# vshiv18/khoice

Measured on AMD Instinct MI355X. Metric: distinct k-mers/sec (k=31, canonical), higher is better.
Workload: dtype u64

## Files before the change

### khoice_amd/csrc/kh_engine.cpp

```cpp
#include <hip/hip_runtime.h>

#include <algorithm>
#include <atomic>
#include <thread>
#include <chrono>
#include <cmath>
#include <memory>
#include <cstdarg>
#include <cstdio>
#include <cstdlib>
#include <cstring>
#include <map>
#include <mutex>
#include <string>
#include <vector>

#include "../../include/khoice_hip.h"
#include "kh_engine.h"
#include "kh_launch.h"
#include "kh_skm_rec.h"

static thread_local std::string g_last_error;

int kh_fail(int code, const char* fmt, ...) {
// ... 344 lines not shown
extern "C" int kh_set_counts(kh_ctx* c, const kh_set* in, uint32_t value, kh_set** out) {
    if (!c || !in || !out) return kh_fail(KH_E_ARG, "kh_set_counts: NULL argument");
    if (value == 0) return kh_fail(KH_E_ARG, "set_counts 0 would empty the database");
    buf_ref(in->kb);
    *out = make_set(in->k, in->n, in->kb, in->koff, nullptr, 0, value, std::max<u32>(value, KH_KMC_DEFAULT_CS));
    return KH_OK;
}

#ifdef KH_STAMPS
void kh_debug_set_stamps(u64* p);
void kh_debug_set_stamps_skm(u64* p);
static void report_stamps(kh_ctx* c, const char* what, DevBuf* sb, u64 nparts) {
    std::vector<u64> h(nparts * 16);
    (void)hipMemcpyAsync(h.data(), sb->p, nparts * 128, hipMemcpyDeviceToHost, c->st);
    (void)hipStreamSynchronize(c->st);
    double sum[16] = {0};
    u64 cnt = 0, tmin = ~0ull, tmax = 0;
    for (u64 q = 0; q < nparts; ++q) {
        const u64* t = &h[q * 16];
        if (!t[0] || !t[8]) continue;
        ++cnt;
        for (int i = 1; i <= 8; ++i) if (t[i] && t[i - 1]) sum[i] += (double)(t[i] - t[i - 1]);
        tmin = std::min(tmin, t[0]);
        tmax = std::max(tmax, t[8]);
    }
    {
        double s9 = 0, s10 = 0, s11 = 0; u64 c9 = 0;
        for (u64 q = 0; q < nparts; ++q) {
            const u64* t = &h[q * 16];
            if (!t[4] || !t[9] || !t[10] || !t[11] || !t[5]) continue;
            ++c9; s9 += (double)(t[9] - t[4]); s10 += (double)(t[10] - t[9]); s11 += (double)(t[11] - t[10]);
        }
        if (c9) fprintf(stderr, "[stamps] %s inside 4-5: first-probe %.0f rounds %.0f stores %.0f (then barrier)\n", what, s9 / c9, s10 / c9, s11 / c9);
    }
    fprintf(stderr, "[stamps] %s parts=%llu span=%.0f cyc | load %.0f count %.0f scan %.0f scatter %.0f insert %.0f walk1 %.0f lookback %.0f walk2 %.0f\n",
            what, (unsigned long long)cnt, (double)(tmax - tmin), sum[1] / cnt, sum[2] / cnt, sum[3] / cnt, sum[4] / cnt,
            sum[5] / cnt, sum[6] / cnt, sum[7] / cnt, sum[8] / cnt);
    {
        std::string line;
        for (int i = 1; i < 16; ++i) {
            double s2 = 0; u64 c2 = 0;
            for (u64 q = 0; q < nparts; ++q) {
                const u64* t = &h[q * 16];
                if (!t[0] || !t[i]) continue;
                ++c2; s2 += (double)((long long)(t[i] - t[0]));
            }
            if (c2) { char b[64]; snprintf(b, sizeof b, " t%d=%.0f(n=%llu)", i, s2 / c2, (unsigned long long)c2); line += b; }
        }
        fprintf(stderr, "[stamps] %s offsets from t0:%s\n", what, line.c_str());
    }
}
#ifdef KH_STAMPS_WG
void kh_debug_set_stamps_skm2(u64* p);
static void dump_wg_ends(kh_ctx* c, DevBuf* sb, u32 grid) {
    const char* path = getenv("KHOICE_WG_DUMP");
    if (!path) return;
    static int call = 0;
    std::vector<u64> h((size_t)grid * 16);
    (void)hipMemcpyAsync(h.data(), sb->p, (size_t)grid * 128, hipMemcpyDeviceToHost, c->st);
    (void)hipStreamSynchronize(c->st);
    FILE* f = fopen(path, "a");
    if (!f) return;
    for (u32 b = 0; b < grid; ++b) {
        const u64* t = &h[(size_t)b * 16];
        fprintf(f, "%d %u %llu %llu %llu %llu %llu %llu\n", call, b, (unsigned long long)t[1], (unsigned long long)t[2],
                (unsigned long long)t[0], (unsigned long long)t[8], (unsigned long long)t[3], (unsigned long long)t[11]);
    }
    fclose(f);
    ++call;
}
#endif
#endif

struct TextStage {
    Tmp d_seq;
    std::vector<const u8*> dev;
    int copy_in(kh_ctx* c, int n, const uint8_t* const* seqs, const uint64_t* lens, int on_device, const int* perm = nullptr) {
        auto in_place = [&](const uint8_t* p) { return on_device && (reinterpret_cast<uintptr_t>(p) & 15) == 0; };
        std::vector<u64> pack_off(n);
        u64 seq_bytes = 0;
        bool need_pack = false;
        for (int i = 0; i < n; ++i) {
            const int t = perm ? perm[i] : i;
            pack_off[i] = seq_bytes;
            seq_bytes += (lens[t] + 15) & ~15ull;
            if (!in_place(seqs[t])) need_pack = true;
        }
        TMP_ALLOC(d_seq, c, need_pack ? seq_bytes + 256 : 256);
        dev.resize(n);
        for (int i = 0; i < n; ++i) {
            const int t = perm ? perm[i] : i;
            if (in_place(seqs[t])) { dev[i] = seqs[t]; continue; }
            dev[i] = d_seq.as<u8>() + pack_off[i];
            if (!lens[t]) continue;
            HIPCHK(hipMemcpyAsync(d_seq.as<u8>() + pack_off[i], seqs[t], lens[t],
                                  on_device ? hipMemcpyDeviceToDevice : hipMemcpyHostToDevice, c->st));
            c->stat.text_packed += lens[t];
        }
        return KH_OK;
    }
};

struct GridBuild {
    kh_ctx* c = nullptr;
    u32 fan = 1;
    u32 cap = 0;
    double s_scale = 1.0;
    u32 wave = 0, nwaves = 1;
    u32 nb = 0, S = 0, nb_total = 0;
    u64 total_pos = 0, bases = 0, key_cap = 0;
// ... 1176 lines not shown
    const u64 lim = (u64)wd.max_coarse * wd.max_fine;
    if (!force_slots && nslots64 > lim) {
        const double per_slot = (double)positions * per_kmer / (double)lim;
        const double s2 = ((double)max_cap2 - 112.0) / per_slot;
        if (s2 >= 1.4 && (!g.two || (double)positions / (double)lim <= 0.75 * (double)wd.table)) {
            nslots64 = lim;
            slack2 = std::min(slack2, s2);
        }
    }
    const u32 max_coarse = nslots64 > lim ? kh_skm_width(true).max_coarse : wd.max_coarse;
    if (nslots64 > (u64)max_coarse * wd.max_fine) {
        if (!table || force_slots) return false;
        nslots64 = (u64)max_coarse * wd.max_fine;
        fuller = true;
    }
    g.nslots = (u32)nslots64;
    g.S = std::max<u32>(1, (g.nslots + max_coarse - 1) / max_coarse);
    g.nb1 = (g.nslots + g.S - 1) / g.S;
    const double recs = (double)positions * per_kmer;
    if (const char* e = getenv("KHOICE_SKM_SLACK")) slack1 = slack2 = std::max(0.01, atof(e));
    const u64 cap1_64 = ((u64)(recs / g.nb1 * slack1) + 2048 + 63) & ~63ull;
    u64 cap2_64 = ((u64)(recs / g.nslots * slack2) + 96 + 15) & ~15ull;
    if (cap2_64 > max_cap2 && !force_slots && !fuller) {
        if ((double)fan + recs / (double)g.nslots <= (double)max_cap2 - 112.0) cap2_64 = max_cap2 & ~15u;
    }
    if (cap2_64 > max_cap2 || cap1_64 > 0x7fffffffull) return false;
    g.cap1 = (u32)cap1_64;
    g.cap2 = (u32)cap2_64;
    g.ugrid = std::min<u32>(g.nslots, wd.union_per_cu * (u32)std::max(1, cus));
    *out = g;
    return true;
}
template <class F> static int timed_launch(kh_ctx* c, int cls, F launch) {
    c->prof_begin(cls);
    launch();
    c->prof_end();
    HIPCHK(hipGetLastError());
    return KH_OK;
}
struct SkmRun {
    kh_ctx* c;
    TagLayout L;
    SkmGeometry g;
    KhSkmJob job;
    struct Layout { size_t ctl, inst, dup, cur1, cur2, claim, ginfo, tags, segs, tiles, bytes; } off{};
    TextStage texts;
    Tmp d_ws, d_reg1, d_reg2, d_spill;
    Pinned pin;
    u8* h_down = nullptr;
    u32 ntiles = 0;
    u64 bases = 0;
    bool staged = false;
    static constexpr u32 spill_cap = 1u << 20, big_cap = 16384u;
#ifdef KH_STAMPS
    Tmp d_stamps;
#endif
    explicit SkmRun(kh_ctx* ctx) : c(ctx), pin{ctx} {}

    void layout(size_t hist_words, int nseq) {
        off.ctl = 8 * hist_words;
        off.inst = off.ctl + 4 * (size_t)KH_SKM_CTL_WORDS;
        off.dup = off.inst + 8 * (size_t)nseq;
        off.cur1 = off.dup + 8 * 64;
        off.cur2 = off.cur1 + 4 * (size_t)KH_SKM_CUR1_STRIDE * g.nb1;
        off.claim = (off.cur2 + 4 * (size_t)g.nslots + 127) & ~(size_t)127;
        off.ginfo = off.claim + 128;
        off.tags = off.ginfo + 256;
        off.segs = off.tags + (((size_t)nseq + 15) & ~(size_t)15);
        off.tiles = off.segs + sizeof(KhSeg) * nseq;
        off.bytes = off.tiles + sizeof(KhTile) * (size_t)std::max<u32>(1, ntiles);
    }
    template <class T> T* dev(size_t o) const { return reinterpret_cast<T*>(d_ws.as<u8>() + o); }
    int read_back(size_t from) {
        HIPCHK(hipMemcpyAsync(h_down + from, d_ws.as<u8>() + from, off.cur1 - from, hipMemcpyDeviceToHost, c->st));
        HIPCHK(hipStreamSynchronize(c->st));
        return KH_OK;
    }
    const u64* h_hist() const { return reinterpret_cast<const u64*>(h_down); }
    const u32* h_ctl() const { return reinterpret_cast<const u32*>(h_down + off.ctl); }
    const u64* h_inst() const { return reinterpret_cast<const u64*>(h_down + off.inst); }
    const u64* h_dup() const { return reinterpret_cast<const u64*>(h_down + off.dup); }
    bool failed() const { return (h_ctl()[KH_SKM_CTL_ERR] & (KH_ERR_CAPACITY | KH_ERR_ORDER)) != 0; }
    template <class F> int settle(size_t from, F listed, bool* declines) {
        *declines = true;
        KHCHK(read_back(from));
        const u32* hc = h_ctl();
        if (hc[KH_SKM_CTL_LISTED] && !failed()) {
            if (hc[KH_SKM_CTL_SPILLED] > spill_cap || hc[KH_SKM_CTL_LISTED] > big_cap) { c->stat.retries++; return KH_OK; }
            KHCHK(listed(hc[KH_SKM_CTL_LISTED]));
            KHCHK(read_back(from));
        }
        if (failed()) { c->stat.retries++; return KH_OK; }
        *declines = false;
        return KH_OK;
    }
    template <class F> void per_text(F f) const {
        for (int i = 0; i < L.nseq; ++i) f(L.perm[i], h_inst()[i], h_inst()[i] - h_dup()[i]);
    }
};
static int skm_prepare(kh_ctx* c, int nseq, const uint8_t* const* seqs, const uint64_t* lens, int on_device,
                       const int* group_of, int ngroups, int k, bool by_group, u32 force_slots, u32 fan_hint, SkmRun* s,
                       u32 table = 0 ) {
    TagLayout* L = &s->L;
    if (!skm_form_k(k)) return KH_OK;
    if ((!by_group && nseq > KH_TAG_MAX_OPS) || ngroups > KH_TAG_MAX_OPS) return KH_OK;
    KHCHK(tag_layout(L, nseq, group_of, ngroups, by_group));
    if (L->nbins > (u32)KH_TAG_MAX_BINS) return KH_OK;
    const u64 positions = kmer_positions(nseq, lens, k, &s->bases);
    if (!skm_plan(k, positions, std::max(L->fan, fan_hint), force_slots, c->cus, &s->g, table)) return KH_OK;
    const SkmGeometry& g = s->g;
    const KhSkmWidth& wd = *g.wd;
    const size_t rec_bytes = wd.rec_bytes;
    const size_t reg1_bytes = rec_bytes * (size_t)g.nb1 * g.cap1, reg2_bytes = rec_bytes * (size_t)g.nslots * g.cap2;
    HIPCHK(hipSetDevice(c->dev));
    {
        size_t free_b = 0, total_b = 0;
        if (hipMemGetInfo(&free_b, &total_b) == hipSuccess &&
            reg1_bytes + reg2_bytes + s->bases + (64u << 20) > free_b + c->pool.cached_bytes)
            return KH_OK;
    }
    hipStream_t st = c->st;

    u32 tile_pos = KH_TILE;
    {
        const u64 want_tiles = 8ull * (u64)std::max(1, c->cus);
        while (tile_pos > (u32)KH_SUBTILE && (positions + tile_pos - 1) / tile_pos < want_tiles) tile_pos >>= 1;
    }
    std::vector<KhSeg> segs(nseq);
    std::vector<KhTile> tiles;
    for (int i = 0; i < nseq; ++i) {
        KhSeg& sg = segs[i];
        memset(&sg, 0, sizeof sg);
        const u64 len = lens[L->perm[i]];
        sg.len = len;
        sg.npos = len >= (u64)k ? len - k + 1 : 0;
        sg.ntiles = (u32)((sg.npos + tile_pos - 1) / tile_pos);
        sg.tile_base = (u32)tiles.size();
        for (u32 t = 0; t < sg.ntiles; ++t) tiles.push_back(KhTile{(u32)i, t});
    }
    const u32 ntiles = s->ntiles = (u32)tiles.size();
    const u32 reps = g.ugrid;
    s->layout((size_t)reps * L->nbins, nseq);
    const SkmRun::Layout& off = s->off;
    const u32 spill_cap = SkmRun::spill_cap;
    TMP_ALLOC(s->d_ws, c, off.bytes);
    TMP_ALLOC(s->d_reg1, c, reg1_bytes);
    TMP_ALLOC(s->d_reg2, c, reg2_bytes);
    TMP_ALLOC(s->d_spill, c, (size_t)spill_cap * (rec_bytes + 4) + (size_t)SkmRun::big_cap * 4);
    const size_t up_bytes = off.bytes - off.ginfo;
    PIN_ALLOC(s->pin, up_bytes + off.cur1 + 64);
    u8* h_up = static_cast<u8*>(s->pin.p);
    s->h_down = h_up + ((up_bytes + 63) & ~(size_t)63);
    c->prof_begin(KC_COPY_IN);
    KHCHK(s->texts.copy_in(c, nseq, seqs, lens, on_device, L->perm.data()));
    for (int i = 0; i < nseq; ++i) segs[i].seq = s->texts.dev[i];
    memcpy(h_up + (off.segs - off.ginfo), segs.data(), sizeof(KhSeg) * nseq);
    if (ntiles) memcpy(h_up + (off.tiles - off.ginfo), tiles.data(), sizeof(KhTile) * (size_t)ntiles);
    L->words(reinterpret_cast<u32*>(h_up), h_up + (off.tags - off.ginfo), group_of);
    HIPCHK(hipMemsetAsync(s->d_ws.b->p, 0, off.ginfo, st));
    HIPCHK(hipMemcpyAsync(s->dev<u8>(off.ginfo), h_up, up_bytes, hipMemcpyHostToDevice, st));
    c->prof_end();

    KhSkmJob& job = s->job;
    job.seg_tag = by_group ? s->dev<const u8>(off.tags) : nullptr;
    job.segs = s->dev<const KhSeg>(off.segs);
    job.tiles = s->dev<const KhTile>(off.tiles);
    job.reg1 = s->d_reg1.as<uint4>();
    job.reg2 = s->d_reg2.as<uint4>();
    job.cur1 = s->dev<u32>(off.cur1);
    job.cur2 = s->dev<u32>(off.cur2);
    job.inst = s->dev<unsigned long long>(off.inst);
    job.dup = s->dev<unsigned long long>(off.dup);
    job.ginfo = s->dev<const u32>(off.ginfo);
    job.hist = s->dev<unsigned long long>(0);
    job.ctl = s->dev<u32>(off.ctl);
    job.claim = s->dev<u32>(off.claim);
    job.tile_pos = tile_pos;
    job.k = k; job.m = g.m; job.w = g.w; job.nmax = g.nmax;
    job.nslots = g.nslots; job.S = g.S; job.nb1 = g.nb1; job.cap1 = g.cap1; job.cap2 = g.cap2;
    job.nbins = L->nbins; job.abase = L->abase; job.reps = reps; job.nops = by_group ? (u32)ngroups : (u32)nseq;
    job.spill_rec = s->d_spill.as<uint4>();
    job.spill_slot = reinterpret_cast<u32*>(s->d_spill.as<u8>() + (size_t)spill_cap * rec_bytes);
    job.big_list = reinterpret_cast<u32*>(s->d_spill.as<u8>() + (size_t)spill_cap * (rec_bytes + 4));
    job.spill_cap = spill_cap;
    job.big_cap = SkmRun::big_cap;
#ifdef KH_STAMPS
    const u64 nst = std::max<u64>(ntiles, g.nslots);
    TMP_ALLOC(s->d_stamps, c, 128 * nst);
    HIPCHK(hipMemsetAsync(s->d_stamps.b->p, 0, 128 * nst, st));
    kh_debug_set_stamps_skm(s->d_stamps.as<u64>());
#endif
    c->prof_begin(KC_SKM_SCATTER);
    wd.scatter(job, ntiles, st);
    c->prof_end();
#ifdef KH_STAMPS
    report_stamps(c, "skm_scatter (second sub-tile: codes / hashes / minima / slots+count / - / append / barrier / -)", s->d_stamps.b, ntiles);
    HIPCHK(hipMemsetAsync(s->d_stamps.b->p, 0, 128 * nst, st));
    kh_debug_set_stamps_skm(nullptr);
#endif
    c->prof_begin(KC_SKM_REGROUP);
    wd.regroup(job, st);
    c->prof_end();
#ifdef KH_STAMPS
    kh_debug_set_stamps_skm(s->d_stamps.as<u64>());
#ifdef KH_STAMPS_WG
    kh_debug_set_stamps_skm2(s->d_stamps.as<u64>());
#endif
#endif
    s->staged = true;
    return KH_OK;
}
static int exp1_skm(kh_ctx* c, const Exp1In& in, uint64_t* within_hist, uint64_t* across_hist, uint64_t* distinct_per_seq,
                    bool* done, bool by_group = false) {
    *done = false;
    SkmRun s(c);
    KHCHK(skm_prepare(c, in.nseq, in.seqs, in.lens, in.on_device, in.group_of, in.ngroups, in.k, by_group, 0, 0, &s));
    if (!s.staged) return KH_OK;
    const TagLayout& L = s.L;
    const SkmGeometry& g = s.g;
    const KhSkmJob& job = s.job;
    hipStream_t st = c->st;
    KHCHK(timed_launch(c, KC_SKM_UNION, [&] { g.wd->unite(job, in.cs, g.ugrid, st); }));
#if defined(KH_STAMPS) && defined(KH_STAMPS_WG)
    dump_wg_ends(c, s.d_stamps.b, g.ugrid);
    kh_debug_set_stamps_skm(nullptr);
    kh_debug_set_stamps_skm2(nullptr);
#elif defined(KH_STAMPS)
    report_stamps(c, "skm_union (scan barrier / owner / expand / insert / barrier / read-out / barrier / flush)", s.d_stamps.b, g.nslots);
    kh_debug_set_stamps_skm(nullptr);
#endif
    if (getenv("KHOICE_SKM_DEBUG")) {
        std::vector<u32> h1(g.nb1), h2(g.nslots);
        HIPCHK(hipMemcpy2DAsync(h1.data(), 4, job.cur1, 4 * (size_t)KH_SKM_CUR1_STRIDE, 4, g.nb1, hipMemcpyDeviceToHost, st));
        HIPCHK(hipMemcpyAsync(h2.data(), job.cur2, 4 * (size_t)g.nslots, hipMemcpyDeviceToHost, st));
        u32 hc[KH_SKM_CTL_WORDS];
        HIPCHK(hipMemcpyAsync(hc, job.ctl, sizeof hc, hipMemcpyDeviceToHost, st));
        HIPCHK(hipStreamSynchronize(st));
        u64 t1 = 0, t2 = 0;
        u32 m1 = 0, m2 = 0;
        for (u32 v : h1) { t1 += v; m1 = std::max(m1, v); }
        for (u32 v : h2) { t2 += v; m2 = std::max(m2, v); }
        fprintf(stderr, "[skm] k=%d m=%d w=%u nmax=%u positions=%llu records=%llu (%.2f k-mers each) nb1=%u S=%u nslots=%u | "
                        "coarse: mean %.0f max %u cap %u | slot: mean %.1f max %u cap %u | tiles %u x %u | expanded: %u k-mers | errors %u spilled %u overfull slots %u multi-subset slots %u tail-wide waves %u\n",
                in.k, g.m, g.w, g.nmax, (unsigned long long)g.positions, (unsigned long long)t1, (double)g.positions / std::max<u64>(1, t1),
                g.nb1, g.S, g.nslots, (double)t1 / g.nb1, m1, g.cap1, (double)t2 / g.nslots, m2, g.cap2, s.ntiles, job.tile_pos,
                hc[KH_SKM_CTL_EXPANDED], hc[KH_SKM_CTL_ERR], hc[KH_SKM_CTL_SPILLED], hc[KH_SKM_CTL_LISTED], g.two ? 0u : hc[KH_SKM_CTL_MULTI], g.two ? 0u : hc[KH_SKM_CTL_TAILWIDE]);
    }
    bool declines = false;
// ... 1920 lines not shown
```

### khoice_amd/csrc/kh_launch.h

```cpp
#pragma once
#include <hip/hip_runtime.h>
#include "kh_common.h"

struct KhSeg {
    const u8* seq;
    u64 len;
    u64 npos;
    u64 thist_base;
    u32 nbuckets;
    u32 bucket_base;
    u32 tile_base;
    u32 ntiles;
    u32 nb_virtual;
    u32 b_first;
};
struct KhTile { u32 seg; u32 tile_in_seg; };

struct KhBucketWork {
    u64 lo;
    u64 out_base;
    u32 n;
    u32 nb;
    u32 b;
    u32 gb;
// ... 89 lines not shown
    uint4* reg2;
    u32* cur1;
    u32* cur2;
    unsigned long long* inst;
    unsigned long long* dup;
    const u32* ginfo;
    unsigned long long* hist;
    u32* ctl;
    u32* claim;
    u32 tile_pos;
    int k, m;
    u32 w;
    u32 nmax;
    u32 nslots, S, nb1, cap1, cap2;
    u32 nbins, abase, reps, nops;
    uint4* spill_rec;
    u32* spill_slot;
    u32* big_list;
    u32 spill_cap, big_cap;
};
struct KhSkmCrossJob {
    unsigned long long* bins;
    u32 pmlo, pmhi;
    u32 ngenomes;
    u32 nbins, reps;
    u32 nlisted;
};
struct KhSkmPivotJob {
    KhSkmCrossJob cj;
    u32 pinfo[KH_TAG_MAX_OPS];
};
constexpr int KH_SKM2_MAX_K = 63;
constexpr u32 KH_SKM2_MAX_COARSE = 512;
constexpr u32 KH_SKM2_MAX_FINE = 1024;
struct KhSkmWidth {
    u32 rec_bytes;
    u32 max_coarse, max_fine;
    u32 max_cap2;
    u32 table;
    u32 union_per_cu, cross_per_cu;
    u32 pivot_per_cu;
    u32 cross_round;
    bool (*supports_w)(u32 w);
    void (*scatter)(const KhSkmJob& job, u32 ntiles, hipStream_t st);
    void (*regroup)(const KhSkmJob& job, hipStream_t st);
    void (*unite)(const KhSkmJob& job, u32 cs, u32 grid, hipStream_t st);
    void (*big)(const KhSkmJob& job, u32 cs, u32 nbig, hipStream_t st);
    void (*cross)(const KhSkmJob& job, const KhSkmCrossJob& cj, u32 grid, hipStream_t st);
    void (*pivot)(const KhSkmJob& job, const KhSkmPivotJob& pj, u32 grid, hipStream_t st);
};
const KhSkmWidth& kh_skm_width1();
const KhSkmWidth& kh_skm_width2();
inline const KhSkmWidth& kh_skm_width(bool two) { return two ? kh_skm_width2() : kh_skm_width1(); }
struct KhSkmPackJob {
    const uint4* reg2;
    const u32* cur2;
    uint4* out_rec;
    u32* out_mask;
    u32* part_cursor;
    u32* slot_count;
    u32* slot_off;
    u32* ctl;
    unsigned long long* dup;
    u64 part_cap;
    u32 cap2, nslots, spp;
    u32 nsub;
};
struct KhSkmCompactJob {
    const uint4* tmp_rec;
    const u32* tmp_mask;
    uint4* out_rec;
    u32* out_mask;
    const u32* cursors;
    u32* slot_off;
    u32* part_n;
    u64 part_cap;
    u32 nslots, spp, nsub, nparts;
};
void kh_launch_skm_pack_compact(const KhSkmCompactJob& job, hipStream_t st);
struct KhSkmPiece {
    const uint4* rec;
    const u32* mask;
    const u32* count;
    const u32* off;
    u32 dup_row;
    u32 join_next;
};
struct KhSkmPhasedJob {
    const KhSkmPiece* pieces;
    unsigned long long* hist;
    u32* ctl;
    unsigned long long* dup;
    u32 npieces, nslots, hist_len, cs;
    u32 share_q8;
    int k;
};
constexpr u32 KH_SKM_PHASED_MAX_DUP_PIECES = 32;
size_t kh_skm_phased_lds_bytes();
void kh_launch_skm_pack(const KhSkmPackJob& job, hipStream_t st);
void kh_launch_skm_phased(const KhSkmPhasedJob& job, u32 grid, hipStream_t st);

#ifndef KH_TUNE_BMP_RANGE_BITS
#define KH_TUNE_BMP_RANGE_BITS 20
#endif
constexpr int KH_BMP_RANGE_BITS = KH_TUNE_BMP_RANGE_BITS;
constexpr int KH_BMP_MAX_K = 12;
// ... 137 lines not shown
```

### khoice_amd/csrc/kh_skm.hip

```cpp
#include <hip/hip_runtime.h>

#include "kh_device.h"
#include "kh_launch.h"

#ifdef KH_STAMPS
__device__ u64* g_skm_stamps = nullptr;
void kh_debug_set_stamps_skm(u64* p) { (void)hipMemcpyToSymbol(HIP_SYMBOL(g_skm_stamps), &p, sizeof p); }
#define SKM_STAMP(idx)                                                                     \
    do {                                                                                   \
        __builtin_amdgcn_sched_barrier(0);                                                 \
        if (threadIdx.x == 0 && g_skm_stamps)                                              \
            g_skm_stamps[((u64)blockIdx.y * gridDim.x + blockIdx.x) * 16 + (idx)] = __builtin_amdgcn_s_memtime(); \
        __builtin_amdgcn_sched_barrier(0);                                                 \
    } while (0)
#else
#define SKM_STAMP(idx) do {} while (0)
#endif

#ifdef KH_MARKS
#define SKM_MARK(name) asm volatile("; ===== MARK " name ::: "memory")
#else
#define SKM_MARK(name) do {} while (0)
#endif
#ifndef KH_TUNE_SKM_SCATTER_PREFETCH
#define KH_TUNE_SKM_SCATTER_PREFETCH 0
#endif
#ifndef KH_TUNE_SKM_SCATTER_WAVES
#define KH_TUNE_SKM_SCATTER_WAVES 3
#endif

#include "kh_skm_device.h"

static size_t kh_skm_scatter_lds_bytes(u32 nb1) {
    const u32 nbk = (nb1 + 3) & ~3u;
    return flush_lds_bytes<SKM_CAP>(nbk) + (size_t)SKM_CW * 4 + (((size_t)SKM_CW * 2 + 15) & ~(size_t)15) + 64 * 4 + 4 * 32 * 4 +
           (size_t)SKM_NT * 8 + 64;
}

template <int WW>
__global__ __launch_bounds__(SKM_NT, KH_TUNE_SKM_SCATTER_WAVES) void k_skm_scatter(const KhSkmJob jb) {
    extern __shared__ __attribute__((aligned(16))) u8 lds_raw[];
    const u32 nbk = (jb.nb1 + 3) & ~3u;
    const FlushLds L = flush_lds<SKM_CAP>(lds_raw, nbk);
    u8* p = lds_raw + flush_lds_bytes<SKM_CAP>(nbk);
    u32* code = reinterpret_cast<u32*>(p);                    p += (size_t)SKM_CW * 4;
    u16* bad16 = reinterpret_cast<u16*>(p);                   p += ((size_t)SKM_CW * 2 + 15) & ~(size_t)15;
    u32* tailh = reinterpret_cast<u32*>(p);                   p += 64 * 4;
    u32* xch = reinterpret_cast<u32*>(p);                     p += 4 * 32 * 4;
    uint2* lrun = reinterpret_cast<uint2*>(p);                p += (size_t)SKM_NT * 8;
    u32* misc = reinterpret_cast<u32*>(p);

    const u32 tid = threadIdx.x, lane = lane_id(), wid = tid >> 6;
    const KhTile t = jb.tiles[blockIdx.x];
    const KhSeg sg = jb.segs[t.seg];
    const u32 rtag = jb.seg_tag ? jb.seg_tag[t.seg] : t.seg;
    const int k = jb.k, m = jb.m;
    const u32 nslots = jb.nslots, S = jb.S, nmax = jb.nmax;
    const u64 smagic = ((1ull << 40) + S - 1) / S;
    const u32 mmask = m >= 16 ? 0xffffffffu : ((1u << (2 * m)) - 1u);
    const u64 tile_pos0 = (u64)t.tile_in_seg * jb.tile_pos;
    const int subtiles = (int)(jb.tile_pos / SKM_SUB);

    for (u32 i = tid; i < nbk; i += SKM_NT) L.bcnt[i] = 0;
    if (tid < 4) misc[tid] = 0;
    u32 staged = 0, tile_recs = 0;

    SkmFetch pre;
#if KH_TUNE_SKM_SCATTER_PREFETCH
    skm_fetch(sg.seq, sg.len, tile_pos0, pre);
#endif
    for (int sub = 0; sub < subtiles; ++sub) {
        const u64 p0 = tile_pos0 + (u64)sub * SKM_SUB;
        if (p0 >= sg.npos) break;
        __syncthreads();
        const bool stamp = sub == 1;
        if (stamp) SKM_STAMP(0);
#if !KH_TUNE_SKM_SCATTER_PREFETCH
        skm_fetch(sg.seq, sg.len, p0, pre);
#endif
        skm_store(pre, code, bad16);
        __syncthreads();
        if (stamp) SKM_STAMP(1);
#if KH_TUNE_SKM_SCATTER_PREFETCH
        if (sub + 1 < subtiles && p0 + SKM_SUB < sg.npos) skm_fetch(sg.seq, sg.len, p0 + SKM_SUB, pre);
#endif
        u32 cw[3];
#pragma unroll
        for (int i = 0; i < 3; ++i) cw[i] = code[2 * tid + i];
        u32 cur[SKM_PPT + WW - 1];
        {
            u32 cv[3], rv[3];
#pragma unroll
            for (int i = 0; i < 3; ++i) { cv[i] = ~cw[i]; rv[i] = revpairs32(cw[i]); }
            const u32 fsh = 32u - 2u * (u32)m;
#pragma unroll
            for (int j = 0; j < (int)SKM_PPT; ++j) {
                const int w = j >> 4, o = j & 15;
                const u32 f = (o ? __builtin_amdgcn_alignbit(rv[w], rv[w + 1], 32 - 2 * o) : rv[w]) >> fsh;
                const u32 r = __builtin_amdgcn_alignbit(cv[w + 1], cv[w], 2 * o) & mmask;
                cur[j] = mmer_hash(f < r ? f : r);
            }
        }
        if (WW > 1) {
            if (tid < 64) {
                const u32 q = SKM_SUB + tid, wq = q >> 4, oq = q & 15u;
                const u32 x = __builtin_amdgcn_alignbit(code[wq + 1], code[wq], 2 * oq) & mmask;
                const u32 f = revpairs32(x) >> (32 - 2 * m);
                const u32 r = (~x) & mmask;
                tailh[tid] = mmer_hash(f < r ? f : r);
            }
            if (lane == 0) {
#pragma unroll
                for (int j = 0; j < WW - 1; ++j) xch[wid * 32 + j] = cur[j];
            }
            __syncthreads();
// ... 103 lines not shown
            if (wm) {
                const u32 base = staged + (u32)__builtin_amdgcn_readlane((int)excl, 0);
                const u32 cnt = (u32)__builtin_amdgcn_readlane((int)incl, 63 - __builtin_clzll(wm));
                __builtin_amdgcn_fence(__ATOMIC_RELEASE, "workgroup");
                __builtin_amdgcn_wave_barrier();
                __builtin_amdgcn_fence(__ATOMIC_ACQUIRE, "workgroup");
                for (u32 r = lane; r < cnt; r += KH_WAVE) {
                    const u32 at = base + r;
                    const uint2 d = dsc[2 * at];
                    const u32 src = (d.x >> 5) & (SKM_NT - 1), s = d.x & 31u;
                    const uint2 li = lrun[src];
                    const u32 n = (d.x >> 16) ? (d.x >> 16) : run_len(li.x, li.y, s);
                    const u32 slot = slot_of(d.y, nslots);
                    const u32 coarse = (u32)(((u64)slot * smagic) >> 40), fine = slot - coarse * S;
                    const u32 bp = src * SKM_PPT + s, sh = 2 * (bp & 15u);
                    const u32* cq = code + (bp >> 4);
                    const u32 c0 = cq[0], c1 = cq[1], c2 = cq[2], c3 = cq[3], c4 = cq[4];
                    const int bits = 2 * ((int)n + k - 1);
                    auto keep = [](u32 x, int b) -> u32 { return b >= 32 ? x : (b <= 0 ? 0u : x & ((1u << b) - 1u)); };
                    const u32 x0 = __builtin_amdgcn_alignbit(c1, c0, sh);
                    const u32 x1 = keep(__builtin_amdgcn_alignbit(c2, c1, sh), bits - 32);
                    const u32 x2 = keep(__builtin_amdgcn_alignbit(c3, c2, sh), bits - 64);
                    const u32 x3 = keep(__builtin_amdgcn_alignbit(c4, c3, sh), bits - 96) | SkmRec1::header(fine, rtag, n);
                    L.stage[at] = make_uint4(x0, x1, x2, x3);
                    L.sid[at] = (u16)coarse;
                    atomicAdd(&L.bcnt[coarse], 1u);
                }
            }
            if (wrote) done = true;
            if (stamp) SKM_STAMP(5);
            const u32 room = SKM_CAP - staged;
            if (total <= room) {
                staged += total;
                if (stamp) SKM_STAMP(6);
                __syncthreads();
                if (stamp) { SKM_STAMP(7); SKM_STAMP(8); }
                break;
            }
            if (tid == 0) misc[2] = 0;
            __syncthreads();
            if (fits && mine) atomicMax(&misc[2], excl + mine);
            __syncthreads();
            const u32 part = misc[2];
            if (stamp) SKM_STAMP(10);
            skm_flush<SKM_NT, SKM_CAP, false>(L, staged + part, jb.nb1, jb.cur1, jb.reg1, jb.cap1, jb.ctl);
            if (stamp) SKM_STAMP(11);
            staged = 0;
        }
    }
    __syncthreads();
    if (staged) skm_flush<SKM_NT, SKM_CAP, false>(L, staged, jb.nb1, jb.cur1, jb.reg1, jb.cap1, jb.ctl);
    if (tid == 0 && misc[1]) atomicAdd(&jb.inst[t.seg], (unsigned long long)misc[1]);
    if (tid == 0 && tile_recs) atomicAdd(jb.ctl + KH_SKM_CTL_RECORDS, tile_recs);
}

#ifndef KH_TUNE_SKM_UE
#define KH_TUNE_SKM_UE 2
#endif
constexpr u32 SKM_UE = KH_TUNE_SKM_UE;
constexpr u32 SKM_OB = SKM_UE == 2 ? 4 : 3;
constexpr u32 SKM_PASSES = SKM_UE == 2 ? 3 : 2;
template <u32 NT, u32 T> struct SkmUnionGeo {
    static constexpr u32 TABLE = T;
    static constexpr u32 T2 = 128;
    static constexpr u32 MAXREC = NT;
    static constexpr u32 MAXCH = SKM_PASSES * NT;
    static constexpr size_t LDS = (size_t)T * 16 + (size_t)T2 * 16 + 1024 + 128 + 256 + (size_t)SKM_HSTRIPE_WORDS * 4 +
                                  (size_t)MAXCH * 2 + (size_t)MAXREC * 4;
    static_assert(MAXREC * 16 <= T * 4, "records are staged in the first half of the key plane");
    static_assert(T2 <= NT && T % 4 == 0, "table planes are cleared 16 bytes at a time");
    static_assert((T & (T - 1u)) == 0u, "table indices wrap by a mask");
};
using SkmUnion = SkmUnionGeo<1024, 4096>;
static_assert(SkmUnion::TABLE == 4096, "the slot geometry and its measurements (skm_plan) are the 4096-entry table's");

__device__ __forceinline__ u32 key_hash2(u32 lo, u32 hi) { return (lo ^ hi) * 0x9E3779B1u; }

struct Skm1Consts {
    u32 kml, kmh;
    u32 fsh;
    u32 tsh;
    u32 tsh_sub;
    bool tsh_high;
    __device__ __forceinline__ explicit Skm1Consts(const int k)
        : kml((u32)kh_mask(2 * k)), kmh((u32)(kh_mask(2 * k) >> 32)), fsh(64u - 2u * (u32)k), tsh(2u * (u32)k - 2u),
          tsh_sub(tsh >= 32u ? tsh - 32u : tsh), tsh_high(tsh >= 32u) {}
};
template <int E, class F>
__device__ __forceinline__ void skm1_expand(const uint4 r0, const u32 first, const Skm1Consts& kc, F&& f) {
    const u64 clo = ((u64)r0.y << 32) | r0.x, chi = ((u64)r0.w << 32) | r0.z;
    const u32 sh = 2u * first;
    const u64 lo = sh ? (clo >> sh) | (chi << (64u - sh)) : clo, hi = chi >> sh;
    const u32 xl = (u32)lo & kc.kml, xh = (u32)(lo >> 32) & kc.kmh;
    const u64 fw = kh_revpairs64(((u64)xh << 32) | xl) >> kc.fsh;
    u32 fl = (u32)fw, fh = (u32)(fw >> 32), rl = ~xl & kc.kml, rh = ~xh & kc.kmh;
    const u32 t = (u32)((lo >> kc.tsh) | (hi << (64u - kc.tsh)));
    const u32 tc = ~t;
#pragma unroll
    for (int e = 0; e < E; ++e) {
        if (e) {
            fh = __builtin_amdgcn_alignbit(fh, fl, 30) & kc.kmh;
            fl = ((fl << 2) | ((t >> (2 * e)) & 3u)) & kc.kml;
            rl = __builtin_amdgcn_alignbit(rh, rl, 2);
            rh >>= 2;
            if (kc.tsh_high) rh |= ((tc >> (2 * e)) & 3u) << kc.tsh_sub; else rl |= ((tc >> (2 * e)) & 3u) << kc.tsh_sub;
        }
        const bool fwd = fh < rh || (fh == rh && fl < rl);
        f((u32)e, fwd ? fl : rl, fwd ? fh : rh);
    }
}
struct SkmClaim1 {
    unsigned long long* tkey;
    u32 okey_off;
    unsigned long long empty, K;
    __device__ __forceinline__ u32 operator()(const bool second, const u32 S) const {
        const unsigned long long o2 = atomicCAS(tkey + (second ? okey_off : 0u) + S, empty, K);
        return o2 == empty ? SKM_FRESH : (o2 == K ? SKM_SAME_KEY : SKM_OTHER_KEY);
    }
};

#if defined(KH_STAMPS) && defined(KH_STAMPS_WG)
#define SKM_USTAMP(idx) do {} while (0)
#define SKM_WGSTAMP(idx)                                                                   \
    do {                                                                                   \
        __builtin_amdgcn_sched_barrier(0);                                                 \
        if (threadIdx.x == 0 && g_skm_stamps) {                                            \
            u64* const sp_ = g_skm_stamps + (u64)blockIdx.x * 16;                          \
            sp_[(idx)] = __builtin_amdgcn_s_memtime();                                     \
            sp_[(idx) + 3] = wall_clock64();                                               \
            if ((idx) == 0) {                                                              \
                sp_[1] = __builtin_amdgcn_s_getreg(4 | (31 << 11));                        \
                sp_[2] = __builtin_amdgcn_s_getreg(20 | (31 << 11));                       \
            }                                                                              \
        }                                                                                  \
        __builtin_amdgcn_sched_barrier(0);                                                 \
    } while (0)
#elif defined(KH_STAMPS)
#define SKM_WGSTAMP(idx) do {} while (0)
#define SKM_USTAMP(idx)                                                                    \
    do {                                                                                   \
        __builtin_amdgcn_sched_barrier(0);                                                 \
        if (threadIdx.x == 0 && g_skm_stamps) g_skm_stamps[(u64)slot * 16 + (idx)] = __builtin_amdgcn_s_memtime(); \
        __builtin_amdgcn_sched_barrier(0);                                                 \
    } while (0)
#else
#define SKM_USTAMP(idx) do {} while (0)
#define SKM_WGSTAMP(idx) do {} while (0)
#endif

#ifndef KH_TUNE_SKM_UNION_LEAN
#define KH_TUNE_SKM_UNION_LEAN 1
#endif
#ifndef KH_TUNE_SKM_UNION_KT
#define KH_TUNE_SKM_UNION_KT 1
#endif
#ifndef KH_TUNE_SKM_UNION_PRIO
#define KH_TUNE_SKM_UNION_PRIO 1
#endif
#ifndef KH_TUNE_SKM_UNION_PRIO_LEVEL
#define KH_TUNE_SKM_UNION_PRIO_LEVEL 1
#endif
#ifndef KH_TUNE_SKM_UNION_COMPACT
#define KH_TUNE_SKM_UNION_COMPACT 0
#endif
#define SKM_UNION_PRIO_UP(bit)   do { if ((KH_TUNE_SKM_UNION_PRIO) & (bit)) __builtin_amdgcn_s_setprio(KH_TUNE_SKM_UNION_PRIO_LEVEL); } while (0)
#define SKM_UNION_PRIO_DOWN(bit) do { if ((KH_TUNE_SKM_UNION_PRIO) & (bit)) __builtin_amdgcn_s_setprio(0); } while (0)
template <u32 NT, u32 T, int KT>
__global__ __launch_bounds__(NT, 8) void k_skm_union(const KhSkmJob jb, u32 cs, u32 first_claimed) {
    extern __shared__ __attribute__((aligned(16))) u8 lds_raw[];
    using G = SkmUnionGeo<NT, T>;
    constexpr u32 T2 = G::T2, NW = NT / 64;
    constexpr u32 T2SH = 25;
    constexpr int E = (int)SKM_UE;
    constexpr u64 EMPTY = ~0ull;
    u8* p = lds_raw;
    unsigned long long* tkey = reinterpret_cast<unsigned long long*>(p);   p += (size_t)T * 8;
    u32* tmlo = reinterpret_cast<u32*>(p);                                 p += (size_t)T * 4;
    u32* tmhi = reinterpret_cast<u32*>(p);                                 p += (size_t)T * 4;
    unsigned long long* okey = reinterpret_cast<unsigned long long*>(p);   p += (size_t)T2 * 8;
    u32* omlo = reinterpret_cast<u32*>(p);                                 p += (size_t)T2 * 4;
    u32* omhi = reinterpret_cast<u32*>(p);                                 p += (size_t)T2 * 4;
    uint4* gtab = reinterpret_cast<uint4*>(p);                             p += 1024;
    u32* scratch = reinterpret_cast<u32*>(p);                              p += 128;
    u32* dupc = reinterpret_cast<u32*>(p);                                 p += 256;
    u32* hstripe = reinterpret_cast<u32*>(p);                              p += (size_t)SKM_HSTRIPE_WORDS * 4;
    u16* owner = reinterpret_cast<u16*>(p);                                p += (size_t)G::MAXCH * 2;
    u32* rmask = reinterpret_cast<u32*>(p);
    uint4* stage = reinterpret_cast<uint4*>(tkey);
    u32* dd = reinterpret_cast<u32*>(tkey) + T;
    const u32 tid0 = threadIdx.x, wid = __builtin_amdgcn_readfirstlane(tid0 >> 6);
    u32 tid = tid0, lane = lane_id();
    const u32 nbins = jb.nbins, cap2 = jb.cap2, nslots = jb.nslots;
    const int k = KT ? KT : jb.k;
    const u32 sshift = nbins <= 72u ? 2u : (nbins <= 144u ? 1u : 0u), smask = (1u << sshift) - 1u;
    auto clear_keys = [&]() {
        uint4* k4 = reinterpret_cast<uint4*>(tkey);
        for (u32 i = tid; i < T / 2; i += NT) k4[i] = make_uint4(0xffffffffu, 0xffffffffu, 0xffffffffu, 0xffffffffu);
    };
#if !(defined(KH_ABLATE) && KH_ABLATE == 3)
    constexpr bool MASKS_SELF_CLEAN = true;
#else
// ... 855 lines not shown
                        if (c < hbins) atomicAdd(&lhist[c], 1u);
                        else atomicAdd(&jb.hist[c], 1ull);
                    }
                }
                if (tid < T2 && ocnt[tid]) {
                    u32 c = ocnt[tid] < jb.cs ? ocnt[tid] : jb.cs;
                    c = c < jb.hist_len - 1u ? c : jb.hist_len - 1u;
                    if (c < hbins) atomicAdd(&lhist[c], 1u);
                    else atomicAdd(&jb.hist[c], 1ull);
                }
                if (tid == 0 && q + 1 == R) scratch[2] = 0;
            }
            __syncthreads();
        }
        if (!R) __syncthreads();
    }
    __syncthreads();
    if (tid0 < hbins && lhist[tid0]) atomicAdd(&jb.hist[tid0], (unsigned long long)lhist[tid0]);
}

template <int WW> static void launch_scatter_w(const KhSkmJob& job, u32 ntiles, size_t lds, hipStream_t st) {
    skm_allow_lds(k_skm_scatter<WW>, lds);
    hipLaunchKernelGGL(k_skm_scatter<WW>, dim3(ntiles), dim3(SKM_NT), lds, st, job);
}
static bool kh_skm_supports_w(u32 w) { return w >= (u32)SKM_WMIN && w <= (u32)SKM_WMAX; }
static void kh_launch_skm_scatter(const KhSkmJob& job, u32 ntiles, hipStream_t st) {
    if (!ntiles) return;
    const size_t lds = kh_skm_scatter_lds_bytes(job.nb1);
    switch (job.w) {
#define SKM_W(WW) case WW: launch_scatter_w<WW>(job, ntiles, lds, st); break;
        SKM_W(5) SKM_W(6) SKM_W(7) SKM_W(8) SKM_W(9) SKM_W(10) SKM_W(11) SKM_W(12) SKM_W(13) SKM_W(14) SKM_W(15) SKM_W(16)
        SKM_W(17) SKM_W(18)
#undef SKM_W
        default: break;
    }
}
static void kh_launch_skm_regroup(const KhSkmJob& job, hipStream_t st) { skm_launch_regroup<SkmRec1>(job, st); }
template <int KT> static void launch_union_k(const KhSkmJob& job, u32 cs, u32 grid, hipStream_t st) {
    const size_t lds = SkmUnion::LDS;
    skm_allow_lds(k_skm_union<1024, 4096, KT>, lds);
    hipLaunchKernelGGL((k_skm_union<1024, 4096, KT>), dim3(grid), dim3(1024), lds, st, job, cs, skm_first_claimed(job.nslots, grid));
}
static void kh_launch_skm_union(const KhSkmJob& job, u32 cs, u32 grid, hipStream_t st) {
    switch (job.k) {
#if KH_TUNE_SKM_UNION_KT
#define SKM_K(KK) case KK: launch_union_k<KK>(job, cs, grid, st); break;
        SKM_K(17) SKM_K(18) SKM_K(19) SKM_K(20) SKM_K(21) SKM_K(22) SKM_K(23) SKM_K(24)
        SKM_K(25) SKM_K(26) SKM_K(27) SKM_K(28) SKM_K(29) SKM_K(30) SKM_K(31) SKM_K(32)
#undef SKM_K
#endif
        default: launch_union_k<0>(job, cs, grid, st); break;
    }
}
void kh_launch_skm_pack(const KhSkmPackJob& job, hipStream_t st) {
    if (!job.nslots) return;
    if (job.cap2 <= 256) {
        hipLaunchKernelGGL(k_skm_pack<256>, dim3(job.nslots), dim3(256), skm_pack_lds_bytes(256), st, job);
    } else if (job.cap2 <= 512) {
        hipLaunchKernelGGL(k_skm_pack<512>, dim3(job.nslots), dim3(512), skm_pack_lds_bytes(512), st, job);
    } else {
        const size_t lds = skm_pack_lds_bytes(1024);
        skm_allow_lds(k_skm_pack<1024>, lds);
        hipLaunchKernelGGL(k_skm_pack<1024>, dim3(job.nslots), dim3(1024), lds, st, job);
    }
}
void kh_launch_skm_pack_compact(const KhSkmCompactJob& job, hipStream_t st) {
    if (!job.nparts || !job.nsub) return;
    const u32 z = job.nparts >= 16 ? 1u : 16u / job.nparts;
    hipLaunchKernelGGL(k_skm_pack_compact, dim3(job.nsub, job.nparts, z), dim3(256), 0, st, job);
}
void kh_launch_skm_phased(const KhSkmPhasedJob& job, u32 grid, hipStream_t st) {
    if (!job.nslots || !grid) return;
    const size_t lds = kh_skm_phased_lds_bytes();
    skm_allow_lds(k_skm_phased, lds);
    hipLaunchKernelGGL(k_skm_phased, dim3(grid), dim3(SKM_PH_NT), lds, st, job);
}
constexpr bool SKM_CROSS1_VGPRS64 = true;
constexpr bool SKM_PIVOT1_VGPRS64 = true;
const KhSkmWidth& kh_skm_width1() {
    static const KhSkmWidth wd = {
        (u32)sizeof(uint4) * SkmRec1::Q, KH_SKM_MAX_COARSE, KH_SKM_MAX_FINE, SkmUnion::MAXREC, SkmUnion::TABLE,
        2u , skm_cross_per_cu<SkmBig1>(SKM_CROSS1_VGPRS64),
        skm_cross_per_cu<SkmBig1>(SKM_PIVOT1_VGPRS64), skm_walk_round<SkmBig1>(),
        kh_skm_supports_w, kh_launch_skm_scatter, kh_launch_skm_regroup, kh_launch_skm_union, skm_launch_big<SkmBig1>,
        skm_launch_cross<SkmBig1>, skm_launch_pivot<SkmBig1>,
    };
    return wd;
}
```

Baseline: 119.0 billion.

## Replace workspace memset/memcpy with kernels and cap histogram replicas

Workspace zeroing and the host-to-device upload are fused into one kernel that reads pinned host memory directly, and read-back becomes a kernel that writes into pinned host memory. This is meant to avoid the fixed cost of separate DMA/blit operations on small transfers. Histogram replication is capped at 8 replicas instead of the union grid size, which shrinks the histogram region that gets zeroed and read back. The cap may add atomic contention, and the kernels move small data over PCIe with zero-copy accesses. Debug stamp macros are also moved so they apply to the scatter kernel.

```diff
diff --git a/khoice_amd/csrc/kh_engine.cpp b/khoice_amd/csrc/kh_engine.cpp
--- a/khoice_amd/csrc/kh_engine.cpp
+++ b/khoice_amd/csrc/kh_engine.cpp
@@ -420,10 +420,11 @@
 }
 #ifdef KH_STAMPS_WG
 void kh_debug_set_stamps_skm2(u64* p);
-static void dump_wg_ends(kh_ctx* c, DevBuf* sb, u32 grid) {
-    const char* path = getenv("KHOICE_WG_DUMP");
+static void dump_wg_ends(kh_ctx* c, DevBuf* sb, u32 grid, bool scatter = false) {
+    const char* path = getenv(scatter ? "KHOICE_WG_DUMP_SCATTER" : "KHOICE_WG_DUMP");
     if (!path) return;
-    static int call = 0;
+    static int calls[2] = {0, 0};
+    int& call = calls[scatter];
     std::vector<u64> h((size_t)grid * 16);
     (void)hipMemcpyAsync(h.data(), sb->p, (size_t)grid * 128, hipMemcpyDeviceToHost, c->st);
     (void)hipStreamSynchronize(c->st);
@@ -1706,6 +1707,7 @@
     u64 bases = 0;
     bool staged = false;
     static constexpr u32 spill_cap = 1u << 20, big_cap = 16384u;
+    static constexpr u32 hist_reps = 8u;
 #ifdef KH_STAMPS
     Tmp d_stamps;
 #endif
@@ -1722,11 +1724,12 @@
         off.tags = off.ginfo + 256;
         off.segs = off.tags + (((size_t)nseq + 15) & ~(size_t)15);
         off.tiles = off.segs + sizeof(KhSeg) * nseq;
-        off.bytes = off.tiles + sizeof(KhTile) * (size_t)std::max<u32>(1, ntiles);
+        off.bytes = (off.tiles + sizeof(KhTile) * (size_t)std::max<u32>(1, ntiles) + 15) & ~(size_t)15;
     }
     template <class T> T* dev(size_t o) const { return reinterpret_cast<T*>(d_ws.as<u8>() + o); }
     int read_back(size_t from) {
-        HIPCHK(hipMemcpyAsync(h_down + from, d_ws.as<u8>() + from, off.cur1 - from, hipMemcpyDeviceToHost, c->st));
+        kh_launch_skm_ws_down(h_down + from, d_ws.as<u8>() + from, off.cur1 - from, c->st);
+        HIPCHK(hipGetLastError());
         HIPCHK(hipStreamSynchronize(c->st));
         return KH_OK;
     }
@@ -1793,7 +1796,7 @@
         for (u32 t = 0; t < sg.ntiles; ++t) tiles.push_back(KhTile{(u32)i, t});
     }
     const u32 ntiles = s->ntiles = (u32)tiles.size();
-    const u32 reps = g.ugrid;
+    const u32 reps = std::min(g.ugrid, SkmRun::hist_reps);
     s->layout((size_t)reps * L->nbins, nseq);
     const SkmRun::Layout& off = s->off;
     const u32 spill_cap = SkmRun::spill_cap;
@@ -1811,8 +1814,8 @@
     memcpy(h_up + (off.segs - off.ginfo), segs.data(), sizeof(KhSeg) * nseq);
     if (ntiles) memcpy(h_up + (off.tiles - off.ginfo), tiles.data(), sizeof(KhTile) * (size_t)ntiles);
     L->words(reinterpret_cast<u32*>(h_up), h_up + (off.tags - off.ginfo), group_of);
-    HIPCHK(hipMemsetAsync(s->d_ws.b->p, 0, off.ginfo, st));
-    HIPCHK(hipMemcpyAsync(s->dev<u8>(off.ginfo), h_up, up_bytes, hipMemcpyHostToDevice, st));
+    kh_launch_skm_ws_init(s->d_ws.b->p, off.ginfo, h_up, up_bytes, st);
+    HIPCHK(hipGetLastError());
     c->prof_end();
 
     KhSkmJob& job = s->job;
@@ -1847,7 +1850,11 @@
     c->prof_begin(KC_SKM_SCATTER);
     wd.scatter(job, ntiles, st);
     c->prof_end();
-#ifdef KH_STAMPS
+#if defined(KH_STAMPS) && defined(KH_STAMPS_WG)
+    dump_wg_ends(c, s->d_stamps.b, ntiles, true);
+    HIPCHK(hipMemsetAsync(s->d_stamps.b->p, 0, 128 * nst, st));
+    kh_debug_set_stamps_skm(nullptr);
+#elif defined(KH_STAMPS)
     report_stamps(c, "skm_scatter (second sub-tile: codes / hashes / minima / slots+count / - / append / barrier / -)", s->d_stamps.b, ntiles);
     HIPCHK(hipMemsetAsync(s->d_stamps.b->p, 0, 128 * nst, st));
     kh_debug_set_stamps_skm(nullptr);
diff --git a/khoice_amd/csrc/kh_launch.h b/khoice_amd/csrc/kh_launch.h
--- a/khoice_amd/csrc/kh_launch.h
+++ b/khoice_amd/csrc/kh_launch.h
@@ -165,6 +165,8 @@
 const KhSkmWidth& kh_skm_width1();
 const KhSkmWidth& kh_skm_width2();
 inline const KhSkmWidth& kh_skm_width(bool two) { return two ? kh_skm_width2() : kh_skm_width1(); }
+void kh_launch_skm_ws_init(void* ws, size_t zero_bytes, const void* up, size_t up_bytes, hipStream_t st);
+void kh_launch_skm_ws_down(void* down, const void* ws, size_t bytes, hipStream_t st);
 struct KhSkmPackJob {
     const uint4* reg2;
     const u32* cur2;
diff --git a/khoice_amd/csrc/kh_skm.hip b/khoice_amd/csrc/kh_skm.hip
--- a/khoice_amd/csrc/kh_skm.hip
+++ b/khoice_amd/csrc/kh_skm.hip
@@ -16,6 +16,38 @@
 #else
 #define SKM_STAMP(idx) do {} while (0)
 #endif
+#if defined(KH_STAMPS) && defined(KH_STAMPS_WG)
+#define SKM_USTAMP(idx) do {} while (0)
+#define SKM_WGSTAMP(idx)                                                                   \
+    do {                                                                                   \
+        __builtin_amdgcn_sched_barrier(0);                                                 \
+        if (threadIdx.x == 0 && g_skm_stamps) {                                            \
+            u64* const sp_ = g_skm_stamps + (u64)blockIdx.x * 16;                          \
+            sp_[(idx)] = __builtin_amdgcn_s_memtime();                                     \
+            sp_[(idx) + 3] = wall_clock64();                                               \
+            if ((idx) == 0) {                                                              \
+                sp_[1] = __builtin_amdgcn_s_getreg(4 | (31 << 11));                        \
+                sp_[2] = __builtin_amdgcn_s_getreg(20 | (31 << 11));                       \
+            }                                                                              \
+        }                                                                                  \
+        __builtin_amdgcn_sched_barrier(0);                                                 \
+    } while (0)
+#elif defined(KH_STAMPS)
+#define SKM_WGSTAMP(idx) do {} while (0)
+#define SKM_USTAMP(idx)                                                                    \
+    do {                                                                                   \
+        __builtin_amdgcn_sched_barrier(0);                                                 \
+        if (threadIdx.x == 0 && g_skm_stamps) g_skm_stamps[(u64)slot * 16 + (idx)] = __builtin_amdgcn_s_memtime(); \
+        __builtin_amdgcn_sched_barrier(0);                                                 \
+    } while (0)
+#else
+#define SKM_USTAMP(idx) do {} while (0)
+#define SKM_WGSTAMP(idx) do {} while (0)
+#endif
+#if defined(KH_STAMPS) && defined(KH_STAMPS_WG)
+#undef SKM_STAMP
+#define SKM_STAMP(idx) do {} while (0)
+#endif
 
 #ifdef KH_MARKS
 #define SKM_MARK(name) asm volatile("; ===== MARK " name ::: "memory")
@@ -61,6 +93,7 @@
     const u64 tile_pos0 = (u64)t.tile_in_seg * jb.tile_pos;
     const int subtiles = (int)(jb.tile_pos / SKM_SUB);
 
+    SKM_WGSTAMP(0);
     for (u32 i = tid; i < nbk; i += SKM_NT) L.bcnt[i] = 0;
     if (tid < 4) misc[tid] = 0;
     u32 staged = 0, tile_recs = 0;
@@ -270,6 +303,10 @@
     if (staged) skm_flush<SKM_NT, SKM_CAP, false>(L, staged, jb.nb1, jb.cur1, jb.reg1, jb.cap1, jb.ctl);
     if (tid == 0 && misc[1]) atomicAdd(&jb.inst[t.seg], (unsigned long long)misc[1]);
     if (tid == 0 && tile_recs) atomicAdd(jb.ctl + KH_SKM_CTL_RECORDS, tile_recs);
+#if defined(KH_STAMPS) && defined(KH_STAMPS_WG)
+    __syncthreads();
+#endif
+    SKM_WGSTAMP(8);
 }
 
 #ifndef KH_TUNE_SKM_UE
@@ -336,35 +373,6 @@
         return o2 == empty ? SKM_FRESH : (o2 == K ? SKM_SAME_KEY : SKM_OTHER_KEY);
     }
 };
-
-#if defined(KH_STAMPS) && defined(KH_STAMPS_WG)
-#define SKM_USTAMP(idx) do {} while (0)
-#define SKM_WGSTAMP(idx)                                                                   \
-    do {                                                                                   \
-        __builtin_amdgcn_sched_barrier(0);                                                 \
-        if (threadIdx.x == 0 && g_skm_stamps) {                                            \
-            u64* const sp_ = g_skm_stamps + (u64)blockIdx.x * 16;                          \
-            sp_[(idx)] = __builtin_amdgcn_s_memtime();                                     \
-            sp_[(idx) + 3] = wall_clock64();                                               \
-            if ((idx) == 0) {                                                              \
-                sp_[1] = __builtin_amdgcn_s_getreg(4 | (31 << 11));                        \
-                sp_[2] = __builtin_amdgcn_s_getreg(20 | (31 << 11));                       \
-            }                                                                              \
-        }                                                                                  \
-        __builtin_amdgcn_sched_barrier(0);                                                 \
-    } while (0)
-#elif defined(KH_STAMPS)
-#define SKM_WGSTAMP(idx) do {} while (0)
-#define SKM_USTAMP(idx)                                                                    \
-    do {                                                                                   \
-        __builtin_amdgcn_sched_barrier(0);                                                 \
-        if (threadIdx.x == 0 && g_skm_stamps) g_skm_stamps[(u64)slot * 16 + (idx)] = __builtin_amdgcn_s_memtime(); \
-        __builtin_amdgcn_sched_barrier(0);                                                 \
-    } while (0)
-#else
-#define SKM_USTAMP(idx) do {} while (0)
-#define SKM_WGSTAMP(idx) do {} while (0)
-#endif
 
 #ifndef KH_TUNE_SKM_UNION_LEAN
 #define KH_TUNE_SKM_UNION_LEAN 1
@@ -1326,6 +1334,26 @@
         default: launch_union_k<0>(job, cs, grid, st); break;
     }
 }
+__global__ __launch_bounds__(256) void k_skm_ws_init(uint4* __restrict__ ws, const u32 zero16, const uint4* __restrict__ up, const u32 up16) {
+    const u32 n = zero16 + up16, step = gridDim.x * 256u;
+    for (u32 i = blockIdx.x * 256u + threadIdx.x; i < n; i += step)
+        ws[i] = i < zero16 ? make_uint4(0u, 0u, 0u, 0u) : up[i - zero16];
+}
+__global__ __launch_bounds__(256) void k_skm_ws_down(unsigned long long* __restrict__ down, const unsigned long long* __restrict__ ws, const u32 n8) {
+    for (u32 i = blockIdx.x * 256u + threadIdx.x; i < n8; i += gridDim.x * 256u) down[i] = ws[i];
+}
+void kh_launch_skm_ws_init(void* ws, size_t zero_bytes, const void* up, size_t up_bytes, hipStream_t st) {
+    const u32 zero16 = (u32)(zero_bytes / 16), up16 = (u32)(up_bytes / 16);
+    if (!(zero16 + up16)) return;
+    const u32 want = (zero16 + up16 + 255u) / 256u, grid = want < 1024u ? want : 1024u;
+    hipLaunchKernelGGL(k_skm_ws_init, dim3(grid), dim3(256), 0, st, static_cast<uint4*>(ws), zero16, static_cast<const uint4*>(up), up16);
+}
+void kh_launch_skm_ws_down(void* down, const void* ws, size_t bytes, hipStream_t st) {
+    const u32 n8 = (u32)(bytes / 8);
+    if (!n8) return;
+    const u32 want = (n8 + 255u) / 256u, grid = want < 64u ? want : 64u;
+    hipLaunchKernelGGL(k_skm_ws_down, dim3(grid), dim3(256), 0, st, static_cast<unsigned long long*>(down), static_cast<const unsigned long long*>(ws), n8);
+}
 void kh_launch_skm_pack(const KhSkmPackJob& job, hipStream_t st) {
     if (!job.nslots) return;
     if (job.cap2 <= 256) {
```

Measured after the change: 122.0 billion, median of 6. 1.03x the previous value.
